# Traneptora/hydrium

Hardware: AMD Instinct MI355X
Metric: Mpixel/s encode (8K RGB, default q) (higher is better)
Workload: dtype f32

## Files before the change

hydrium_amd/csrc/hip/kernels.hip:

```cpp
#include <hip/hip_runtime.h>
#include <stdint.h>

#include "hydk_common.h"
#include <atomic>
#include <type_traits>

#pragma clang fp contract(off)

namespace {

constexpr int kThreads = 256;
#ifndef HYDK_K1_WAVES
#define HYDK_K1_WAVES 4
#endif
#ifndef HYDK_K1_GATHER
#define HYDK_K1_GATHER 0x10
#endif
#ifndef HYDK_K1_WAVELOCAL
#define HYDK_K1_WAVELOCAL 1
#endif
#ifndef HYDK_K1_SKIP
#define HYDK_K1_SKIP 0
#endif
#ifndef HYDK_K1_ILP
#define HYDK_K1_ILP 2
#endif
#ifndef HYDK_K1_TRIM
#define HYDK_K1_TRIM 0
#endif
#ifndef HYDK_K1_CHANSEQ
#define HYDK_K1_CHANSEQ 0
#endif
#ifndef HYDK_CHAIN_PROBE
#define HYDK_CHAIN_PROBE 0
#endif
#ifndef HYDK_LANE_STEP
#define HYDK_LANE_STEP 1
#endif
#ifndef HYDK_LANE_PIPE
#define HYDK_LANE_PIPE 2
#endif
#ifndef HYDK_CHAIN_PRIO
#define HYDK_CHAIN_PRIO 3
#endif
#ifndef HYDK_LANE_TAB_GLOBAL
#define HYDK_LANE_TAB_GLOBAL 0
#endif
#ifndef HYDK_CHAIN_LDS_MIN
#define HYDK_CHAIN_LDS_MIN 0
#endif
#ifndef HYDK_LANE_NC9_PROBE
#define HYDK_LANE_NC9_PROBE 9
#endif
#ifndef HYDK_CHAIN_HOG
#define HYDK_CHAIN_HOG 0
#endif
#ifndef HYDK_K1_PRIO
#define HYDK_K1_PRIO 0
#endif
constexpr int kS0Block = 72;
constexpr int kS0Chan = 32 * kS0Block;
constexpr int kDbgPitch = 2048;

constexpr float kA = (float)0.17338, kB = (float)0.146984, kC = (float)0.0982119, kD = (float)0.0344874;
constexpr float kE = (float)0.16332, kF = (float)0.0676495, kG = (float)0.125;

constexpr float kDct[7][8] = {
    {kA, kB, kC, kD, -kD, -kC, -kB, -kA},
    {kE, kF, -kF, -kE, -kE, -kF, kF, kE},
    {kB, -kD, -kA, -kC, kC, kA, kD, -kB},
    {kG, -kG, -kG, kG, kG, -kG, -kG, kG},
    {kC, -kA, kD, kB, -kB, -kD, kA, -kC},
    {kF, -kE, kE, -kF, -kF, kE, -kE, kF},
    {kD, -kC, kB, -kA, kA, -kB, kC, -kD},
};

__device__ const uint8_t kZigzag[8][8] = {
     {0, 2, 3, 9, 10, 20, 21, 35},
     {1, 4, 8, 11, 19, 22, 34, 36},
     {5, 7, 12, 18, 23, 33, 37, 48},
     {6, 13, 17, 24, 32, 38, 47, 49},
     {14, 16, 25, 31, 39, 46, 50, 57},
     {15, 26, 30, 40, 45, 51, 56, 58},
     {27, 29, 41, 44, 52, 55, 59, 62},
     {28, 42, 43, 53, 54, 60, 61, 63},
};

struct NibbleMasks {
    unsigned long long m[8][2][16];
    constexpr NibbleMasks() : m() {
        constexpr uint8_t zz[8][8] = {{0, 2, 3, 9, 10, 20, 21, 35},   {1, 4, 8, 11, 19, 22, 34, 36},  {5, 7, 12, 18, 23, 33, 37, 48},
                                      {6, 13, 17, 24, 32, 38, 47, 49}, {14, 16, 25, 31, 39, 46, 50, 57}, {15, 26, 30, 40, 45, 51, 56, 58},
                                      {27, 29, 41, 44, 52, 55, 59, 62}, {28, 42, 43, 53, 54, 60, 61, 63}};
        for (int kh = 0; kh < 8; kh++)
            for (int half = 0; half < 2; half++)
                for (int pat = 0; pat < 16; pat++) {
                    unsigned long long v = 0;
                    for (int b = 0; b < 4; b++)
                        if (pat >> b & 1)
                            v |= 1ull << zz[4 * half + b][kh];
                    m[kh][half][pat] = v;
                }
    }
};
__device__ const NibbleMasks kNibbleMasks = NibbleMasks();

__device__ const int16_t kQuantWeight[3][64] = {
    {1969, 1969, 1969, 1962, 1969, 1962, 1655, 1885, 1885, 1655, 1397, 1610, 1704, 1610, 1397, 1178,
     1368, 1494, 1494, 1368, 1178, 994,  1159, 1289, 1340, 1289, 1159, 994,  839,  980,  1104, 1178,
     1178, 1104, 980,  839,  829,  941,  1023, 1054, 1023, 941,  829,  800,  881,  928,  928,  881,
     800,  755,  809,  829,  809,  755,  663,  731,  731,  663,  491,  524,  491,  349,  349,  239},
    {280, 280, 280, 279, 280, 279, 245, 271, 271, 245, 214, 239, 250, 239, 214, 188,
     211, 226, 226, 211, 188, 164, 185, 201, 207, 201, 185, 164, 144, 163, 178, 188,
     188, 178, 163, 144, 143, 157, 168, 172, 168, 157, 143, 139, 150, 156, 156, 150,
     139, 133, 140, 143, 140, 133, 125, 129, 129, 125, 116, 118, 116, 107, 107, 98},
    {256, 147, 147, 85, 117, 85, 60, 78, 78, 60, 43, 56, 63, 56, 43, 43,
     43,  48,  48,  43, 43,  42, 43, 43, 43, 43, 43, 42, 29, 41, 43, 43,
     43,  43,  41,  29, 29,  37, 43, 43, 43, 37, 29, 27, 33, 36, 36, 33,
     27,  24,  27,  29, 27,  24, 20, 22, 22, 20, 15, 16, 15, 10, 10, 7},
};

__device__ const uint8_t kNnzCtx[64] = {
    0,   0,   31,  62,  62,  93,  93,  93,  93,  123, 123, 123, 123, 152, 152, 152, 152, 152, 152, 152, 152, 180,
    180, 180, 180, 180, 180, 180, 180, 180, 180, 180, 180, 206, 206, 206, 206, 206, 206, 206, 206, 206, 206, 206,
    206, 206, 206, 206, 206, 206, 206, 206, 206, 206, 206, 206, 206, 206, 206, 206, 206, 206, 206, 206,
};

constexpr float kLfShift[3] = {8192.f, 1024.f, 512.f};


constexpr float kUnit16 = 1.0f / (65536 - 1.0f);

__device__ __forceinline__ float linearize(float x) {
    if (x <= 0.0404482362771082f)
        return 0.07739938080495357f * x;
    return 0.003094300919832f + x * (-0.009982599f + x * (0.72007737769f + 0.2852804880f * x));
}

__device__ __forceinline__ float bias_curve(float v) {
    const float x = v + 0.0037930732552754493f;
    float z = __uint_as_float(0x548c39cbu - __float_as_uint(x) / 3u);
    z *= 1.5015480449f - 0.534850249f * x * z * z * z;
    z *= 1.333333985f - 0.33333333f * x * z * z * z;
    return 1.0f / z - 0.155954f;
}

__device__ __forceinline__ uint32_t to_u16(float x) {
    const int y = (int)(x * 65535.f + 0.5f);
    return (uint32_t)(y < 0 ? 0 : y > 65535 ? 65535 : y);
}

constexpr int kXybFastRcp = 0, kXybIeeeDiv = 1, kXybGather = 2;
constexpr int kXybFastRcpRegs = 3, kXybIeeeDivRegs = 4;
constexpr int xyb_arith(int xm) { return xm == kXybFastRcpRegs ? kXybFastRcp : xm == kXybIeeeDivRegs ? kXybIeeeDiv : xm; }
constexpr int xyb_gmask(int xm) { return xm == kXybFastRcpRegs || xm == kXybIeeeDivRegs ? 0 : HYDK_K1_GATHER; }

__device__ __forceinline__ uint32_t input_lut16_eval(uint32_t i, int linear_light) {
    const float f = (float)i * kUnit16;
    return (uint32_t)(int)((linear_light ? f : linearize(f)) * 65535.f + 0.5f);
}
constexpr uint32_t kDarkMax = 2650;
constexpr int kCurveBoth = 0, kCurveNone = 1, kCurveCubic = 2;
template <int CURVE>
__device__ __forceinline__ uint32_t input_lut16_eval_as(uint32_t i) {
    const float f = (float)i * kUnit16;
    const float y = CURVE == kCurveNone ? f : CURVE == kCurveCubic
        ? 0.003094300919832f + f * (-0.009982599f + f * (0.72007737769f + 0.2852804880f * f)) : linearize(f);
    return (uint32_t)(int)(y * 65535.f + 0.5f);
}
__device__ __forceinline__ uint32_t div3(uint32_t u) { return __umulhi(u, 0x55555556u); }
template <int XMODE>
__device__ __forceinline__ float bias_lut_eval(uint32_t i) {
    if (xyb_arith(XMODE) == kXybIeeeDiv)
        return bias_curve((float)i * kUnit16);
    const float x = (float)i * kUnit16 + 0.0037930732552754493f;
    float z = __uint_as_float(0x548c39cbu - div3(__float_as_uint(x)));
    z *= 1.5015480449f - 0.534850249f * x * z * z * z;
    z *= 1.333333985f - 0.33333333f * x * z * z * z;
    const float r0 = __builtin_amdgcn_rcpf(z);
    const float r1 = __builtin_fmaf(r0, __builtin_fmaf(-z, r0, 1.0f), r0);
    return r1 - 0.155954f;
}

#define HYDK_GLOBAL(T, p) ((__attribute__((address_space(1))) T *)(p))
template <int CURVE, int N>
__device__ __forceinline__ void input_lut16_eval_n(const uint32_t (&i)[N], uint32_t (&o)[N]) {
    float f[N], y[N];
#pragma unroll
    for (int k = 0; k < N; k++)
        f[k] = (float)i[k] * kUnit16;
    if (CURVE == kCurveNone) {
#pragma unroll
        for (int k = 0; k < N; k++)
            y[k] = f[k];
    } else {
#pragma unroll
        for (int k = 0; k < N; k++)
            y[k] = 0.2852804880f * f[k];
#pragma unroll
        for (int k = 0; k < N; k++)
            y[k] = 0.72007737769f + y[k];
#pragma unroll
        for (int k = 0; k < N; k++)
            y[k] = f[k] * y[k];
#pragma unroll
        for (int k = 0; k < N; k++)
            y[k] = -0.009982599f + y[k];
#pragma unroll
        for (int k = 0; k < N; k++)
            y[k] = f[k] * y[k];
#pragma unroll
        for (int k = 0; k < N; k++)
            y[k] = 0.003094300919832f + y[k];
        if (CURVE == kCurveBoth) {
#pragma unroll
            for (int k = 0; k < N; k++)
                y[k] = f[k] <= 0.0404482362771082f ? 0.07739938080495357f * f[k] : y[k];
        }
    }
#pragma unroll
    for (int k = 0; k < N; k++)
        y[k] = y[k] * 65535.f;
#pragma unroll
    for (int k = 0; k < N; k++)
        y[k] = y[k] + 0.5f;
#pragma unroll
    for (int k = 0; k < N; k++)
        o[k] = (uint32_t)(int)y[k];
}

template <int XMODE, int N>
__device__ __forceinline__ void bias_lut_eval_n(const uint32_t (&i)[N], float (&o)[N]) {
    if (xyb_arith(XMODE) == kXybIeeeDiv) {
#pragma unroll
        for (int k = 0; k < N; k++)
            o[k] = bias_curve((float)i[k] * kUnit16);
        return;
    }
    float x[N], z[N], t[N];
#pragma unroll
    for (int k = 0; k < N; k++)
        x[k] = (float)i[k] * kUnit16;
#pragma unroll
    for (int k = 0; k < N; k++)
        x[k] = x[k] + 0.0037930732552754493f;
#pragma unroll
    for (int k = 0; k < N; k++)
        z[k] = __uint_as_float(0x548c39cbu - div3(__float_as_uint(x[k])));
#pragma unroll
    for (int k = 0; k < N; k++)
        t[k] = 0.534850249f * x[k];
#pragma unroll
    for (int r = 0; r < 3; r++)
#pragma unroll
        for (int k = 0; k < N; k++)
            t[k] = t[k] * z[k];
#pragma unroll
    for (int k = 0; k < N; k++)
        t[k] = 1.5015480449f - t[k];
#pragma unroll
    for (int k = 0; k < N; k++)
        z[k] = z[k] * t[k];
#pragma unroll
    for (int k = 0; k < N; k++)
        t[k] = 0.33333333f * x[k];
#pragma unroll
    for (int r = 0; r < 3; r++)
#pragma unroll
        for (int k = 0; k < N; k++)
            t[k] = t[k] * z[k];
#pragma unroll
    for (int k = 0; k < N; k++)
        t[k] = 1.333333985f - t[k];
#pragma unroll
    for (int k = 0; k < N; k++)
        z[k] = z[k] * t[k];
#pragma unroll
    for (int k = 0; k < N; k++)
        t[k] = __builtin_amdgcn_rcpf(z[k]);
#pragma unroll
    for (int k = 0; k < N; k++)
        x[k] = __builtin_fmaf(-z[k], t[k], 1.0f);
#pragma unroll
    for (int k = 0; k < N; k++)
        t[k] = __builtin_fmaf(t[k], x[k], t[k]);
#pragma unroll
    for (int k = 0; k < N; k++)
        o[k] = t[k] - 0.155954f;
}

__device__ __forceinline__ uint32_t umad24(uint32_t c, uint32_t x, uint32_t acc) {
    uint32_t d;
    asm("v_mad_u32_u24 %0, %1, %2, %3" : "=v"(d) : "s"(c), "v"(x), "v"(acc));
    return d;
}

template <int XMODE>
__device__ __forceinline__ void lms_mix_u16(uint32_t r, uint32_t g, uint32_t b, const float *bias_lut, float &X,
                                            float &Y, float &B) {
    constexpr bool LUTS = XMODE == kXybGather;
    const uint32_t bb = __umul24(5112u, b);
    const uint32_t il = umad24(19661u, r, umad24(40761u, g, bb)) >> 16;
    const uint32_t im = umad24(15073u, r, umad24(45350u, g, bb)) >> 16;
    const uint32_t is = umad24(15953u, r, umad24(13419u, g, __umul24(36163u, b))) >> 16;
    float l, m, s;
    if (LUTS) {
        l = bias_lut[il];
        m = bias_lut[im];
        s = bias_lut[is];
    } else {
        const auto *gl = HYDK_GLOBAL(const float, bias_lut);
        l = (xyb_gmask(XMODE) & 8) ? gl[il] : bias_lut_eval<XMODE>(il);
        m = (xyb_gmask(XMODE) & 16) ? gl[im] : bias_lut_eval<XMODE>(im);
        s = (xyb_gmask(XMODE) & 32) ? gl[is] : bias_lut_eval<XMODE>(is);
    }
    Y = (l + m) * 0.5f;
    X = Y - m;
    B = s - Y;
}

__device__ __forceinline__ bool lms_mix_f32(float r, float g, float b, int linear_light, float &X, float &Y,
                                            float &B) {
    const bool finite = ((__float_as_uint(r) & 0x7f800000u) != 0x7f800000u) &&
                        ((__float_as_uint(g) & 0x7f800000u) != 0x7f800000u) &&
                        ((__float_as_uint(b) & 0x7f800000u) != 0x7f800000u);
    if (!linear_light) {
        r = linearize(r);
        g = linearize(g);
        b = linearize(b);
    }
    const float l = bias_curve(0.3f * r + 0.622f * g + 0.078f * b);
    const float m = bias_curve(0.23f * r + 0.692f * g + 0.078f * b);
    const float s = bias_curve(0.243423f * r + 0.204767f * g + 0.55181f * b);
    Y = (l + m) * 0.5f;
    X = Y - m;
    B = s - Y;
    return finite;
}

__device__ __forceinline__ void dct8(const float (&x)[8], float (&o)[8]) {
    float dc = x[0];
#pragma unroll
    for (int n = 1; n < 8; n++)
        dc += x[n];
    o[0] = dc * 0.125f;
#pragma unroll
    for (int k = 1; k < 8; k++) {
        if (k == 4) {
            float acc = x[0];
#pragma unroll
            for (int n = 1; n < 8; n++)
                acc = kDct[3][n] > 0 ? acc + x[n] : acc - x[n];
            o[k] = acc * 0.125f;
            continue;
        }
        float acc = x[0] * kDct[k - 1][0];
#pragma unroll
        for (int n = 1; n < 8; n++)
            acc += x[n] * kDct[k - 1][n];
        o[k] = acc;
    }
}

__device__ __forceinline__ uint32_t pack_signed(int v) {
    const uint32_t w = (uint32_t)v;
    return (w << 1) ^ (0u - (w >> 31));
}

template <int FMT>
struct SampleOf;
template <>
struct SampleOf<HYDK_FMT_U8> {
    typedef uint8_t type;
};
template <>
struct SampleOf<HYDK_FMT_U16> {
    typedef uint16_t type;
};
template <>
struct SampleOf<HYDK_FMT_F32> {
    typedef float type;
};

}

#define HYDK_URGENT() __builtin_amdgcn_s_setprio(3)

#define HYDK_DPP(v, ctrl, rmask) ((uint32_t)__builtin_amdgcn_update_dpp(0, (int)(v), (ctrl), (rmask), 0xF, false))
__device__ __forceinline__ uint32_t scan16_inclusive(uint32_t v) {
    v += HYDK_DPP(v, 0x111, 0xF);
    v += HYDK_DPP(v, 0x112, 0xF);
    v += HYDK_DPP(v, 0x114, 0xF);
    v += HYDK_DPP(v, 0x118, 0xF);
    return v;
}
__device__ __forceinline__ uint32_t scan64_inclusive(uint32_t v) {
    v = scan16_inclusive(v);
    v += HYDK_DPP(v, 0x142, 0xA);
    v += HYDK_DPP(v, 0x143, 0xC);
    return v;
}

__device__ __forceinline__ uint32_t or_reduce8(uint32_t v) {
    v |= (uint32_t)__builtin_amdgcn_update_dpp(0, (int)v, 0xB1, 0xF, 0xF, false);
    v |= (uint32_t)__builtin_amdgcn_update_dpp(0, (int)v, 0x4E, 0xF, 0xF, false);
    v |= (uint32_t)__builtin_amdgcn_update_dpp(0, (int)v, 0x141, 0xF, 0xF, false);
    return v;
}

template <int FMT>
__device__ __forceinline__ void store_record(void *tok, uint32_t at, uint32_t token, uint32_t cluster, uint32_t symbol,
                                             uint32_t rbits, uint32_t residue) {
    if (FMT == HYDK_FMT_F32)
        ((uint64_t *)tok)[at] = ((uint64_t)residue << 32) | HYDK_REC_LO(token, cluster, rbits);
    else {
#if HYDK_K1_TRIM
        const uint32_t off = at * 4u;
        *(HYDK_GLOBAL(uint32_t, (char *)tok + off)) = HYDK_REC32(symbol, rbits, residue);
#else
        HYDK_GLOBAL(uint32_t, tok)[at] = HYDK_REC32(symbol, rbits, residue);
#endif
    }
}

template <int FMT>
__device__ __forceinline__ int trunc_as_reference(float x) {
    const int q = (int)x;
    if (FMT != HYDK_FMT_F32)
        return q;
    return x < 2147483648.0f ? q : (int)0x80000000u;
}

#define HYDK_K1_OCCUPANCY __launch_bounds__(kThreads, HYDK_K1_WAVES)
template <int FMT, int XMODE, int STORE = HYDK_STORE_F32>
__global__ HYDK_K1_OCCUPANCY void k_transform_tokenize(const HydkLfJob *__restrict__ jobs, uint32_t *status, uint2 *part_info,
                                                       int plog) {
    static_assert(STORE == HYDK_STORE_F32 || (STORE == HYDK_STORE_NV12 ? FMT == HYDK_FMT_U8 : FMT == HYDK_FMT_F32),
                  "the float class has the half-precision storage forms, the 8-bit class NV12");
    constexpr bool NV12 = STORE == HYDK_STORE_NV12;
    constexpr bool HALF = STORE != HYDK_STORE_F32 && !NV12;
    typedef typename std::conditional<HALF, uint16_t, typename SampleOf<FMT>::type>::type sample_t;
    constexpr bool LUTS = XMODE == kXybGather;
    constexpr int kWords = FMT == HYDK_FMT_U8 ? 6 : 12;
#if HYDK_K1_PRIO
    __builtin_amdgcn_s_setprio(HYDK_K1_PRIO);
#endif
    const unsigned bid = blockIdx.x >> plog, part = blockIdx.x & ((1u << plog) - 1u);
    const HydkLfJob job = jobs[bid >> 6];
    if (job.fmt != FMT || (FMT != HYDK_FMT_F32 && job.use_luts != xyb_arith(XMODE) + (NV12 ? HYDK_VARIANT_NV12 : 0)) ||
        (FMT == HYDK_FMT_F32 && job.storage != (uint32_t)STORE))
        return;
    if ((int)(bid & 63) >= job.gcols * job.grows)
        return;
    if (FMT == HYDK_FMT_F32 && job.rec_bytes != 8) {
        if (threadIdx.x == 0) {
            atomicOr(status, HYDK_STATUS_LAYOUT);
            job.sym_count[bid & 63] = 0;
            job.rbits_total[bid & 63] = 0;
            if (plog)
                part_info[blockIdx.x] = uint2{0u, 0u};
        }
        return;
    }

#if HYDK_K1_CHANSEQ
    static_assert(HYDK_K1_WAVELOCAL, "the channels share one row-pass buffer: a wavefront must read only what it wrote");
    typedef typename std::conditional<FMT == HYDK_FMT_F32, int32_t, int16_t>::type coef_t;
    constexpr int kQBlock = 64;
    __shared__ float s_rowpass[kS0Chan];
    __shared__ __attribute__((aligned(16))) coef_t s_q[3 * 32 * kQBlock];
#else
    __shared__ float s_rowpass[3 * kS0Chan];
#endif
    __shared__ uint32_t s_boff[33];
    __shared__ uint32_t s_rbits;
    constexpr int kHistW = FMT == HYDK_FMT_F32 ? 72 : (int)HYDK_REC32_TOKENS;
    __shared__ uint32_t s_hist[HYDK_MAX_CLUSTERS * kHistW];
    __shared__ uint16_t s_lut8[256];
    __shared__ uint8_t s_nnz3[64];
    __shared__ uint16_t s_jinfo[64];
    __shared__ uint4 s_seg[32 * 3];
    __shared__ uint32_t s_blen[32];
    __shared__ __attribute__((aligned(16))) float s_wq[3 * 64];

    const int t = threadIdx.x;
    const int lane = t & 63;
    const int wave = t >> 6;
    const int g = (int)(bid & 63);
    const int gx = g % job.gcols, gy = g / job.gcols;
    const int px0 = gx << 8, py0 = gy << 8;
    const int gw = min(256, job.width - px0), gh = min(256, job.height - py0);
    const int gbw = (gw + 7) >> 3, gbh = (gh + 7) >> 3;

    for (int i = t; i < HYDK_MAX_CLUSTERS * kHistW; i += kThreads)
        s_hist[i] = 0;
    if (FMT == HYDK_FMT_U8)
        s_lut8[t] = job.in_lut8[t];
    if (t < 64) {
        const int j = t;
        s_nnz3[t] = kNnzCtx[t] % 3;
        ((uint8_t *)s_jinfo)[2 * kZigzag[t >> 3][t & 7]] = HYDK_K1_CHANSEQ ? (uint8_t)(((t & 7) << 3) | (t >> 3)) : (uint8_t)t;
        ((uint8_t *)s_jinfo)[2 * t + 1] = (uint8_t)((j < 2 ? 0 : j < 16 ? j - 1 : j < 32 ? 15 + ((j - 16) >> 1) : 23 + ((j - 32) >> 2)) % 3);
    }
    if (t < 192)
        s_wq[t] = (float)kQuantWeight[t >> 6][kZigzag[t & 7][(t >> 3) & 7]];

    const int cb = t >> 3, kh = t & 7;
    const uint32_t nib_row = (uint32_t)kh * (uint32_t)sizeof(kNibbleMasks.m[0]);
    const int coef_cl_lo = job.scheme == 0 ? 3 : job.scheme == 3 ? 0 : 1;

    const bool packed = !NV12 && job.pixel_stride == 3 &&
                        (const char *)job.src[1] == (const char *)job.src[0] + sizeof(sample_t) &&
                        (const char *)job.src[2] == (const char *)job.src[0] + 2 * sizeof(sample_t) &&
                        (((uintptr_t)job.src[0] | (uintptr_t)(job.row_stride * (long long)sizeof(sample_t))) & 3) == 0 &&
                        FMT != HYDK_FMT_F32;

#if HYDK_K1_WAVELOCAL
    const int ar = lane >> 3, ab = (wave << 3) | (lane & 7);
#else
    const int ar = t >> 5, ab = t & 31;
#endif
    int hrun = 0;
    if (HALF) {
        const bool rows4 = ((job.row_stride * 2) & 3) == 0;
        if (!(job.per_sample & 1u) && job.pixel_stride == 3 && rows4 && ((uintptr_t)job.src[0] & 3) == 0 &&
            (const char *)job.src[1] == (const char *)job.src[0] + 2 && (const char *)job.src[2] == (const char *)job.src[0] + 4)
            hrun = 1;
        else if (!(job.per_sample & 2u) && job.pixel_stride == 1 && rows4 &&
                 (((uintptr_t)job.src[0] | (uintptr_t)job.src[1] | (uintptr_t)job.src[2]) & 3) == 0)
            hrun = 2;
    }
    const bool hfast = HALF && hrun != 0 && ab < gbw && ab * 8 + 8 <= gw;
    const bool nvrun = NV12 && (((uintptr_t)job.src[0] | (uintptr_t)job.src[1] | (uintptr_t)job.row_stride) & 3) == 0;
    const HydkYuvMatrix yuv = hydk_yuv_matrix(NV12 ? (int)job.matrix : 0);
    const bool fast = (NV12 ? nvrun : packed) && ab < gbw && ab * 8 + 8 <= gw;
    uint32_t nxt[kWords];
#pragma unroll
    for (int k = 0; k < kWords; k++)
        nxt[k] = 0;
    auto prefetch = [&](int s) {
        if (HALF) {
            if (hfast && s * 8 + ar < gh) {
                const long long row = (long long)(py0 + s * 8 + ar) * job.row_stride;
                if (hrun == 1) {
                    const char *p = (const char *)job.src[0] + (row + (long long)(px0 + ab * 8) * 3) * 2;
#pragma unroll
                    for (int k = 0; k < 12; k++)
                        nxt[k] = HYDK_GLOBAL(const uint32_t, p)[k];
                } else {
#pragma unroll
                    for (int c = 0; c < 3; c++) {
                        const char *p = (const char *)job.src[c] + (row + (long long)(px0 + ab * 8)) * 2;
#pragma unroll
                        for (int k = 0; k < 4; k++)
                            nxt[4 * c + k] = HYDK_GLOBAL(const uint32_t, p)[k];
                    }
                }
            }
            return;
        }
        if (NV12) {
            if (fast && s * 8 + ar < gh) {
                const long long y = py0 + s * 8 + ar, x = px0 + ab * 8;
                const char *py = (const char *)job.src[0] + y * job.row_stride + x;
                const char *pc = (const char *)job.src[1] + (y >> 1) * job.row_stride + x;
#pragma unroll
                for (int k = 0; k < 2; k++) {
                    nxt[k] = HYDK_GLOBAL(const uint32_t, py)[k];
                    nxt[2 + k] = HYDK_GLOBAL(const uint32_t, pc)[k];
                }
            }
            return;
        }
        if (fast && s * 8 + ar < gh) {
            const uint32_t *p = (const uint32_t *)((const char *)job.src[0] +
                                                   ((long long)(py0 + s * 8 + ar) * job.row_stride +
                                                    (long long)(px0 + ab * 8) * 3) * (long long)sizeof(sample_t));
#pragma unroll
            for (int k = 0; k < kWords; k++)
                nxt[k] = HYDK_GLOBAL(const uint32_t, p)[k];
        }
    };
    const int s_per = (gbh + (1 << plog) - 1) >> plog;
    const int s_first = (int)part * s_per, s_end = min(gbh, s_first + s_per);
    const uint32_t tok_room = job.tok_cap >> plog;
    prefetch(s_first);

    void *const tok = (char *)job.tokens + (size_t)g * job.tok_cap * job.rec_bytes + (size_t)part * tok_room * (FMT == HYDK_FMT_F32 ? 8u : 4u);
    uint32_t goff = 0;
    uint32_t rb_sum = 0;
    bool overflowed = false;
    if (t == 0)
        s_rbits = 0;
    bool bad_sample = false;
    __syncthreads();

    for (int s = s_first; s < s_end; s++) {
        float xv[8], yv[8], bv[8];
        if (ab < gbw) {
            const int y = py0 + s * 8 + ar;
            const int x0 = px0 + ab * 8;
            const bool row_ok = s * 8 + ar < gh;
            auto float_pixel = [&](float fr, float fg, float fb, float &X, float &Y, float &B) {
                if (job.bad_slot) {
                    const bool ir = (__float_as_uint(fr) & 0x7f800000u) == 0x7f800000u;
                    const bool ig = (__float_as_uint(fg) & 0x7f800000u) == 0x7f800000u;
                    const bool ib = (__float_as_uint(fb) & 0x7f800000u) == 0x7f800000u;
                    bad_sample = bad_sample || ir || ig || ib;
                    fr = ir ? 0.0f : fr;
                    fg = ig ? 0.0f : fg;
                    fb = ib ? 0.0f : fb;
                }
                if (!lms_mix_f32(fr, fg, fb, job.linear_light, X, Y, B))
                    bad_sample = true;
            };
            if (HALF && hfast) {
#pragma unroll
                for (int i = 0; i < 8; i++) {
                    xv[i] = yv[i] = bv[i] = 0.0f;
                    if (row_ok) {
                        float f[3];
#pragma unroll
                        for (int ch = 0; ch < 3; ch++) {
                            const int ki = i * 3 + ch, kp = ch * 8 + i;
                            const uint32_t wi = nxt[ki >> 1] >> (16 * (ki & 1)), wp = nxt[kp >> 1] >> (16 * (kp & 1));
                            f[ch] = __uint_as_float(hydk_widen_half(STORE, (hrun == 1 ? wi : wp) & 0xFFFFu));
                        }
                        float_pixel(f[0], f[1], f[2], xv[i], yv[i], bv[i]);
                    }
                }
                prefetch(s + 1);
            } else if (fast) {
                uint32_t cvt[kWords];
                if (NV12) {
#pragma unroll
                    for (int k = 0; k < kWords; k++)
                        cvt[k] = 0;
#pragma unroll
                    for (int i = 0; i < 8; i++) {
                        uint32_t rgb[3];
                        hydk_yuv_to_rgb(yuv, (nxt[i >> 2] >> (8 * (i & 3))) & 0xFF, (nxt[2 + (i >> 2)] >> (8 * (i & 2))) & 0xFF,
                                        (nxt[2 + (i >> 2)] >> (8 * (i & 2) + 8)) & 0xFF, rgb);
#pragma unroll
                        for (int ch = 0; ch < 3; ch++) {
                            const int si = i * 3 + ch;
                            cvt[si >> 2] |= rgb[ch] << (8 * (si & 3));
                        }
                    }
                }
                uint32_t(&w)[kWords] = NV12 ? cvt : nxt;
                int curve = kCurveBoth;
                if (FMT == HYDK_FMT_U16 && !LUTS) {
                    if (job.linear_light)
                        curve = kCurveNone;
                    else {
                        typedef uint16_t u16x2 __attribute__((ext_vector_type(2)));
                        u16x2 mn = __builtin_bit_cast(u16x2, w[0]);
#pragma unroll
                        for (int k = 1; k < kWords; k++)
                            mn = __builtin_elementwise_min(mn, __builtin_bit_cast(u16x2, w[k]));
                        const bool dark = row_ok && (uint32_t)(mn.x < mn.y ? mn.x : mn.y) <= kDarkMax;
                        curve = __builtin_amdgcn_ballot_w64(dark) ? kCurveBoth : kCurveCubic;
                    }
                }
                auto row_to_xyb = [&](auto curve_tag) {
                    constexpr int CURVE = decltype(curve_tag)::value;
#if HYDK_K1_ILP
                    if (FMT != HYDK_FMT_F32 && !LUTS) {
                        constexpr int P = HYDK_K1_ILP;
#pragma unroll
                        for (int i0 = 0; i0 < 8; i0 += P) {
                            uint32_t smp[3 * P], lin[3 * P], idx[3 * P];
                            float bia[3 * P];
                            if (FMT == HYDK_FMT_U8) {
#pragma unroll
                                for (int k = 0; k < 3 * P; k++) {
                                    const int si = i0 * 3 + k;
                                    lin[k] = s_lut8[(w[si >> 2] >> (8 * (si & 3))) & 0xFF];
                                }
                            } else {
#pragma unroll
                                for (int k = 0; k < 3 * P; k++) {
                                    const int si = i0 * 3 + k;
                                    smp[k] = (w[si >> 1] >> (16 * (si & 1))) & 0xFFFF;
                                }
                                input_lut16_eval_n<CURVE, 3 * P>(smp, lin);
                            }
#pragma unroll
                            for (int q = 0; q < P; q++) {
                                const uint32_t r = lin[3 * q], g = lin[3 * q + 1], b = lin[3 * q + 2];
                                const uint32_t bb = __umul24(5112u, b);
                                idx[3 * q] = umad24(19661u, r, umad24(40761u, g, bb)) >> 16;
                                idx[3 * q + 1] = umad24(15073u, r, umad24(45350u, g, bb)) >> 16;
                                idx[3 * q + 2] = umad24(15953u, r, umad24(13419u, g, __umul24(36163u, b))) >> 16;
                            }
                            constexpr auto gathered = [](int k) constexpr { return ((xyb_gmask(XMODE) >> 3) >> (k % 3) & 1) != 0; };
                            constexpr int NG = [&]() constexpr { int n = 0; for (int k = 0; k < 3 * P; k++) n += gathered(k); return n; }();
                            if (NG == 0)
                                bias_lut_eval_n<XMODE, 3 * P>(idx, bia);
                            else {
                                const auto *gl = HYDK_GLOBAL(const float, job.bias_lut);
                                constexpr int NE = 3 * P - NG > 0 ? 3 * P - NG : 1;
                                uint32_t eidx[NE];
                                float eb[NE];
                                int n = 0;
#pragma unroll
                                for (int k = 0; k < 3 * P; k++) {
                                    if (gathered(k))
                                        bia[k] = gl[idx[k]];
                                    else
                                        eidx[n++] = idx[k];
                                }
                                if (NG < 3 * P)
                                    bias_lut_eval_n<XMODE, NE>(eidx, eb);
                                n = 0;
#pragma unroll
                                for (int k = 0; k < 3 * P; k++)
                                    if (!gathered(k))
                                        bia[k] = eb[n++];
                            }
#pragma unroll
                            for (int q = 0; q < P; q++) {
                                const float Y = (bia[3 * q] + bia[3 * q + 1]) * 0.5f;
                                yv[i0 + q] = Y;
                                xv[i0 + q] = Y - bia[3 * q + 1];
                                bv[i0 + q] = bia[3 * q + 2] - Y;
                            }
                        }
                        return;
                    }
#endif
#pragma unroll
                    for (int i = 0; i < 8; i++) {
                        uint32_t rgb[3];
#pragma unroll
                        for (int ch = 0; ch < 3; ch++) {
                            const int si = i * 3 + ch;
                            if (FMT == HYDK_FMT_U8)
                                rgb[ch] = s_lut8[(w[si >> 2] >> (8 * (si & 3))) & 0xFF];
                            else {
                                const uint32_t v = (w[si >> 1] >> (16 * (si & 1))) & 0xFFFF;
                                rgb[ch] = LUTS ? (uint32_t)job.in_lut16[v] : (xyb_gmask(XMODE) >> ch & 1) ? (uint32_t)HYDK_GLOBAL(const uint16_t, job.in_lut16)[v] : input_lut16_eval_as<CURVE>(v);
                            }
                        }
                        if (HYDK_K1_SKIP & 2) {
                            xv[i] = __uint_as_float(0x3f000000u | w[(i * 3) >> 1]);
                            yv[i] = __uint_as_float(0x3f000000u | w[(i * 3 + 1) >> 1]);
                            bv[i] = __uint_as_float(0x3f000000u | w[(i * 3 + 2) >> 1]);
                            continue;
                        }
                        lms_mix_u16<XMODE>(rgb[0], rgb[1], rgb[2], job.bias_lut, xv[i], yv[i], bv[i]);
                    }
                };
                if (row_ok) {
                    if (curve == kCurveCubic)
                        row_to_xyb(std::integral_constant<int, kCurveCubic>());
                    else if (curve == kCurveNone)
                        row_to_xyb(std::integral_constant<int, kCurveNone>());
                    else
                        row_to_xyb(std::integral_constant<int, kCurveBoth>());
                } else {
#pragma unroll
                    for (int i = 0; i < 8; i++)
                        xv[i] = yv[i] = bv[i] = 0.0f;
                }
                prefetch(s + 1);
            } else {
                const int nvalid = row_ok ? min(8, gw - ab * 8) : 0;
#pragma unroll
                for (int i = 0; i < 8; i++) {
                    xv[i] = yv[i] = bv[i] = 0.0f;
                    if (i < nvalid) {
                        const long long off = (long long)y * job.row_stride + (long long)(x0 + i) * job.pixel_stride;
                        const long long offc = NV12 ? (long long)(y >> 1) * job.row_stride + (long long)((x0 + i) & ~1) : off;
                        const sample_t sr = ((const sample_t *)job.src[0])[off];
                        const sample_t sg = ((const sample_t *)job.src[1])[offc];
                        const sample_t sb = ((const sample_t *)job.src[2])[offc];
                        if (FMT == HYDK_FMT_F32) {
                            float fr, fg, fb;
                            if (HALF) {
                                fr = __uint_as_float(hydk_widen_half(STORE, (uint32_t)sr));
                                fg = __uint_as_float(hydk_widen_half(STORE, (uint32_t)sg));
                                fb = __uint_as_float(hydk_widen_half(STORE, (uint32_t)sb));
                            } else {
                                fr = (float)sr, fg = (float)sg, fb = (float)sb;
                            }
                            float_pixel(fr, fg, fb, xv[i], yv[i], bv[i]);
                        } else {
                            uint32_t rgb[3] = {(uint32_t)sr, (uint32_t)sg, (uint32_t)sb};
                            if (NV12)
                                hydk_yuv_to_rgb(yuv, (uint32_t)sr, (uint32_t)sg, (uint32_t)sb, rgb);
#pragma unroll
                            for (int ch = 0; ch < 3; ch++) {
                                if (FMT == HYDK_FMT_U8)
                                    rgb[ch] = s_lut8[rgb[ch]];
                                else
                                    rgb[ch] = LUTS ? job.in_lut16[rgb[ch]] : input_lut16_eval(rgb[ch], job.linear_light);
                            }
                            lms_mix_u16<XMODE>(rgb[0], rgb[1], rgb[2], job.bias_lut, xv[i], yv[i], bv[i]);
                        }
                    }
                }
            }
            if (job.dbg_xyb) {
                float *d = job.dbg_xyb + (size_t)y * kDbgPitch + x0;
#pragma unroll
                for (int i = 0; i < 8; i++) {
                    d[i] = xv[i];
                    d[(size_t)kDbgPitch * kDbgPitch + i] = yv[i];
                    d[(size_t)2 * kDbgPitch * kDbgPitch + i] = bv[i];
                }
            }
#if !HYDK_K1_CHANSEQ
            float o[8];
            float *dst = s_rowpass + ab * kS0Block + ar * 8;
            dct8(xv, o);
#pragma unroll
            for (int k = 0; k < 8; k++)
                dst[k] = o[k];
            dct8(yv, o);
#pragma unroll
            for (int k = 0; k < 8; k++)
                dst[kS0Chan + k] = o[k];
            dct8(bv, o);
#pragma unroll
            for (int k = 0; k < 8; k++)
                dst[2 * kS0Chan + k] = o[k];
#endif
        }
#define HYDK_K1_WAVE_SYNC()                                                                                      \
    do {                                                                                                         \
        __builtin_amdgcn_fence(__ATOMIC_RELEASE, "wavefront");                                                   \
        __builtin_amdgcn_wave_barrier();                                                                         \
        __builtin_amdgcn_fence(__ATOMIC_ACQUIRE, "wavefront");                                                   \
    } while (0)
#if HYDK_K1_CHANSEQ
#elif HYDK_K1_WAVELOCAL
        HYDK_K1_WAVE_SYNC();
#else
        __syncthreads();
#endif

        unsigned long long msk[3] = {0, 0, 0};
        int32_t lf_int[3] = {0, 0, 0};
        auto column_pass = [&](const int c) __attribute__((always_inline)) {
                float col[8], v[8];
                float *src = s_rowpass + (HYDK_K1_CHANSEQ ? 0 : c * kS0Chan) + cb * kS0Block + kh;
#pragma unroll
                for (int n = 0; n < 8; n++)
                    col[n] = src[n * 8];
                dct8(col, v);
                if (job.dbg_dct) {
                    float *d = job.dbg_dct + (size_t)c * kDbgPitch * kDbgPitch +
                               (size_t)(py0 + s * 8 + kh) * kDbgPitch + px0 + cb * 8;
#pragma unroll
                    for (int kv = 0; kv < 8; kv++)
                        d[kv] = v[kv];
                }
                uint32_t nlo = 0, nhi = 0;
                int q[8];
                const float4 w03 = *(const float4 *)&s_wq[c * 64 + kh * 8], w47 = *(const float4 *)&s_wq[c * 64 + kh * 8 + 4];
                const float wq[8] = {w03.x, w03.y, w03.z, w03.w, w47.x, w47.y, w47.z, w47.w};
#pragma unroll
                for (int kv = 0; kv < 8; kv++) {
                    const float scaled = v[kv] * wq[kv] * 5.0f;
                    int qq = trunc_as_reference<FMT>(scaled);
                    const bool nz = (FMT == HYDK_FMT_F32 ? !(__builtin_fabsf(scaled) < 2.0f) : __builtin_fabsf(scaled) >= 2.0f) &&
                                    !(kv == 0 && kh == 0);
                    qq = nz ? qq : 0;
                    q[kv] = qq;
                    if (kv < 4)
                        nlo |= nz ? 8u << kv : 0u;
                    else
                        nhi |= nz ? 8u << (kv - 4) : 0u;
#if !HYDK_K1_CHANSEQ
                    ((int *)src)[kv * 8] = qq;
#endif
                }
#if HYDK_K1_CHANSEQ
                {
                    coef_t *const dq = s_q + (c * 32 + cb) * kQBlock + kh * 8;
                    if (FMT == HYDK_FMT_F32) {
                        *(int4 *)dq = int4{q[0], q[1], q[2], q[3]};
                        *(int4 *)(dq + 4) = int4{q[4], q[5], q[6], q[7]};
                    } else {
                        const uint32_t k0 = 0x05040100u;
                        *(uint4 *)dq = uint4{__builtin_amdgcn_perm((uint32_t)q[1], (uint32_t)q[0], k0), __builtin_amdgcn_perm((uint32_t)q[3], (uint32_t)q[2], k0),
                                             __builtin_amdgcn_perm((uint32_t)q[5], (uint32_t)q[4], k0), __builtin_amdgcn_perm((uint32_t)q[7], (uint32_t)q[6], k0)};
                    }
                }
#endif
                if (job.dbg_quant) {
                    int32_t *d = job.dbg_quant + (size_t)c * kDbgPitch * kDbgPitch +
                                 (size_t)(py0 + s * 8 + kh) * kDbgPitch + px0 + cb * 8;
#pragma unroll
                    for (int kv = 0; kv < 8; kv++)
                        d[kv] = q[kv];
                }
                const char *const nib = (const char *)&kNibbleMasks.m[0][0][0];
                if (!(HYDK_K1_SKIP & 4))
                msk[c] = *(const unsigned long long *)(nib + (nib_row | nlo)) | *(const unsigned long long *)(nib + (nib_row | 128u | nhi));
                lf_int[c] = trunc_as_reference<FMT>(v[0] * kLfShift[c]);
        };
#if HYDK_K1_CHANSEQ
        {
#pragma unroll
            for (int c = 0; c < 3; c++) {
                if (ab < gbw) {
                    float o[8];
                    float *dst = s_rowpass + ab * kS0Block + ar * 8;
                    if (c == 0)
                        dct8(xv, o);
                    else if (c == 1)
                        dct8(yv, o);
                    else
                        dct8(bv, o);
#pragma unroll
                    for (int k = 0; k < 8; k++)
                        dst[k] = o[k];
                }
                HYDK_K1_WAVE_SYNC();
                if (!(HYDK_K1_SKIP & 8) && cb < gbw)
                    column_pass(c);
                HYDK_K1_WAVE_SYNC();
            }
        }
#endif
        if (!(HYDK_K1_SKIP & 8) && cb < gbw) {
#if !HYDK_K1_CHANSEQ
#pragma unroll
            for (int c = 0; c < 3; c++)
                column_pass(c);
#endif
            if (kh == 0) {
#pragma unroll
                for (int c = 0; c < 3; c++)
                    HYDK_GLOBAL(int32_t, job.dc)[(size_t)c * HYDK_DC_PITCH * HYDK_DC_PITCH + (size_t)((py0 >> 3) + s) * HYDK_DC_PITCH + (px0 >> 3) + cb] = lf_int[c];
            }
#if HYDK_K1_TRIM & 2
            {
                typedef unsigned long long u64;
                u64 *const cell = (u64 *)&s_seg[cb * 3];
                if (kh == 0) {
                    cell[0] = 0;
                    cell[2] = 0;
                    cell[4] = 0;
                }
                __builtin_amdgcn_wave_barrier();
                constexpr int at[3] = {2, 0, 4};
#pragma unroll
                for (int c = 0; c < 3; c++) {
                    __hip_atomic_fetch_or((uint32_t *)&cell[at[c]], (uint32_t)msk[c], __ATOMIC_RELAXED, __HIP_MEMORY_SCOPE_WORKGROUP);
                    __hip_atomic_fetch_or((uint32_t *)&cell[at[c]] + 1, (uint32_t)(msk[c] >> 32), __ATOMIC_RELAXED, __HIP_MEMORY_SCOPE_WORKGROUP);
                }
                __builtin_amdgcn_wave_barrier();
                if (kh == 0) {
#pragma unroll
                    for (int c = 0; c < 3; c++)
                        msk[c] = cell[at[c]];
                }
            }
#else
#pragma unroll
            for (int c = 0; c < 3 && !(HYDK_K1_SKIP & 4); c++) {
                const uint32_t lo = or_reduce8((uint32_t)msk[c]), hi = or_reduce8((uint32_t)(msk[c] >> 32));
                msk[c] = ((unsigned long long)hi << 32) | lo;
            }
#endif
        }
        const uint32_t nY = 1u + (msk[1] ? 63u - (uint32_t)__clzll(msk[1]) : 0u);
        const uint32_t nX = 1u + (msk[0] ? 63u - (uint32_t)__clzll(msk[0]) : 0u);
        const uint32_t nB = 1u + (msk[2] ? 63u - (uint32_t)__clzll(msk[2]) : 0u);
        if (kh == 0) {
            s_blen[cb] = cb < gbw ? nY | (nX << 8) | (nB << 16) : 0u;
#if HYDK_K1_CHANSEQ
            const uint32_t base = (uint32_t)(cb * kQBlock), chan_pitch = 32u * kQBlock;
#else
            const uint32_t base = (uint32_t)(cb * kS0Block), chan_pitch = (uint32_t)kS0Chan;
#endif
            s_seg[cb * 3 + 0] = make_uint4((uint32_t)msk[1], (uint32_t)(msk[1] >> 32), nY | ((uint32_t)__popcll(msk[1]) << 8), base + chan_pitch);
            s_seg[cb * 3 + 1] = make_uint4((uint32_t)msk[0], (uint32_t)(msk[0] >> 32), nX | ((uint32_t)__popcll(msk[0]) << 8), base);
            s_seg[cb * 3 + 2] = make_uint4((uint32_t)msk[2], (uint32_t)(msk[2] >> 32), nB | ((uint32_t)__popcll(msk[2]) << 8), base + 2 * chan_pitch);
        }
        __syncthreads();

        {
            const uint32_t len3 = s_blen[lane & 31];
            const uint32_t mine = (len3 & 0xffu) + ((len3 >> 8) & 0xffu) + (len3 >> 16);
            uint32_t inc = scan16_inclusive(mine);
            inc += HYDK_DPP(inc, 0x142, 0xA);
            s_boff[(lane & 31) + 1] = inc;
            if (lane == 0)
                s_boff[0] = 0;
            __builtin_amdgcn_wave_barrier();
        }
        const uint32_t strip_total = s_boff[32];

        {
            overflowed = overflowed || goff + strip_total > tok_room;
            static_assert(kThreads == 256, "run lengths are computed with shifts");
            const uint32_t per = strip_total >> 8, extra = strip_total & 255u;
            uint32_t p = (uint32_t)t * per + min((uint32_t)t, extra);
            const uint32_t pend = overflowed ? 0u : p + per + ((uint32_t)t < extra ? 1u : 0u);
            if (!(HYDK_K1_SKIP & 1) && p < pend) {
                uint32_t b = 0;
#pragma unroll
                for (uint32_t step = 16; step; step >>= 1)
                    b += s_boff[b + step] <= p ? step : 0u;
                uint32_t j = p - s_boff[b];
                const uint32_t len = s_blen[b];
                uint32_t visit = 0;
                if (j >= (len & 0xffu)) {
                    j -= len & 0xffu;
                    visit = 1;
                    if (j >= ((len >> 8) & 0xffu)) {
                        j -= (len >> 8) & 0xffu;
                        visit = 2;
                    }
                }
                uint32_t seg_at = b * 3u + visit;
                uint4 seg = s_seg[seg_at];
                uint32_t n = seg.z & 0xffu, nz_total = seg.z >> 8;
                const unsigned long long m = ((unsigned long long)seg.y << 32) | seg.x;
                uint32_t remaining = nz_total - (uint32_t)__popcll(m & ((1ull << j) - 1ull));
                uint32_t prev = j <= 1u ? (uint32_t)(nz_total <= 4u) : (uint32_t)(m >> (j - 1u)) & 1u;
                const uint32_t coef_base = (uint32_t)coef_cl_lo;
                const uint32_t prev_mask = job.scheme <= 1 ? 1u : 0u, ctx_mask = job.scheme == 0 ? 6u : 0u;
                const uint32_t count_mask = job.scheme == 0 ? 3u : 0u;
                for (; p < pend; p++) {
                    const uint32_t ji = s_jinfo[j];
#if HYDK_K1_CHANSEQ
                    const int coef = (int)s_q[seg.w + (ji & 0xffu)];
#else
                    const int coef = ((const int *)s_rowpass)[seg.w + (ji & 0xffu)];
#endif
                    const bool is_count = j == 0u;
                    const uint32_t value = is_count ? nz_total : pack_signed(coef);
                    const uint32_t u = visit + (uint32_t)s_nnz3[remaining & 63u] + (ji >> 8);
                    const uint32_t cluster = is_count ? (visit & count_mask)
                                                      : coef_base + (prev & prev_mask) + ((0x1248u >> (u + u)) & ctx_mask);
                    uint32_t token, rbits, residue;
                    if (FMT != HYDK_FMT_F32) {
                        const uint32_t fb = __float_as_uint((float)value) >> 22;
                        const bool big = value >= 16u;
                        token = big ? fb - 246u : value;
                        rbits = big ? (fb >> 1) - 128u : 0u;
                        residue = __builtin_amdgcn_ubfe(value, 0u, rbits);
                    } else if (value < 16) {
                        token = value;
                        rbits = 0;
                        residue = 0;
                    } else {
                        const int nb = 30 - __clz((int)value);
                        rbits = (uint32_t)nb;
                        residue = value & ((1u << nb) - 1u);
                        token = 16u + (((uint32_t)(nb - 3) << 1) | ((value >> nb) & 1u));
                    }
#if HYDK_K1_TRIM
                    const uint32_t bin = umad24(cluster, (uint32_t)kHistW, FMT == HYDK_FMT_F32 ? min(token, (uint32_t)kHistW - 1u) : token);
#else
                    const uint32_t bin = cluster * kHistW + (FMT == HYDK_FMT_F32 ? min(token, (uint32_t)kHistW - 1u) : token);
#endif
                    store_record<FMT>(tok, goff + p, token, cluster, bin, rbits, residue);
                    rb_sum += rbits;
                    atomicAdd(&s_hist[bin], 1u);
                    const uint32_t here = coef != 0 ? 1u : 0u;
                    remaining -= here;
                    prev = is_count ? (uint32_t)(nz_total <= 4u) : here;
                    if (++j == n) {
                        seg_at++;
                        visit = visit == 2u ? 0u : visit + 1u;
                        seg = s_seg[seg_at];
                        n = seg.z & 0xffu;
                        nz_total = remaining = seg.z >> 8;
                        j = 0;
                    }
                }
            }
        }
        goff += strip_total;
        __syncthreads();
    }

    __syncthreads();
    uint32_t top_token = 0;
    for (int i = t; i < HYDK_MAX_CLUSTERS * kHistW; i += kThreads) {
        const uint32_t v = s_hist[i];
        if (v) {
            atomicAdd(&job.hist[(i / kHistW) * HYDK_ALPHABET + i % kHistW], v);
            top_token = max(top_token, (uint32_t)(i % kHistW) + 1u);
        }
    }
#pragma unroll
    for (int d = 32; d; d >>= 1)
        top_token = max(top_token, (uint32_t)__shfl_xor((int)top_token, d));
    if (lane == 0 && top_token)
        atomicMax(job.alpha_max, top_token);
#pragma unroll
    for (int d = 32; d; d >>= 1)
        rb_sum += (uint32_t)__shfl_xor((int)rb_sum, d);
    if (lane == 0)
        atomicAdd(&s_rbits, rb_sum);
    __syncthreads();
    if (t == 0) {
        const uint32_t count = overflowed || HYDK_K1_SKIP ? 0u : goff;
        if (plog) {
            part_info[blockIdx.x] = uint2{count, s_rbits};
        } else {
            job.sym_count[g] = count;
            job.rbits_total[g] = s_rbits;
        }
        if (overflowed)
            atomicOr(status, HYDK_STATUS_TOKENS);
    }
    if (FMT == HYDK_FMT_F32 && bad_sample) {
        if (job.bad_slot)
            atomicOr(job.bad_slot, 1u);
        else
            atomicOr(status, HYDK_STATUS_BAD_SAMPLE);
    }
}

#include "lf_huffman.h"

__global__ __launch_bounds__(kThreads) void k_join_parts(const HydkLfJob *__restrict__ jobs, const uint2 *part_info, int plog,
                                                         uint32_t *status) {
    const HydkLfJob job = jobs[blockIdx.x >> 6];
    const int g = blockIdx.x & 63;
    if (g >= job.gcols * job.grows)
        return;
    const uint32_t parts = 1u << plog, room = job.tok_cap >> plog, wpr = job.fmt == HYDK_FMT_F32 ? 2u : 1u;
    uint32_t *const base = (uint32_t *)((char *)job.tokens + (size_t)g * job.tok_cap * job.rec_bytes);
    bool bogus = false;
    uint2 p0 = part_info[(size_t)blockIdx.x * parts];
    if (p0.x > room) {
        p0 = uint2{0u, 0u};
        bogus = true;
    }
    uint32_t total = p0.x, rbits = p0.y;
    for (uint32_t q = 1; q < parts; q++) {
        uint2 pi = part_info[(size_t)blockIdx.x * parts + q];
        if (pi.x > room) {
            pi = uint2{0u, 0u};
            bogus = true;
        }
        const uint32_t *src = base + (size_t)q * room * wpr;
        uint32_t *dst = base + (size_t)total * wpr;
        const uint32_t words = pi.x * wpr;
        if (dst != src) {
            constexpr uint32_t kPer = 8;
            for (uint32_t at = 0; at < words; at += kPer * kThreads) {
                uint32_t v[kPer];
#pragma unroll
                for (uint32_t k = 0; k < kPer; k++) {
                    const uint32_t i = at + k * kThreads + threadIdx.x;
                    v[k] = i < words ? src[i] : 0u;
                }
                __syncthreads();
#pragma unroll
                for (uint32_t k = 0; k < kPer; k++) {
                    const uint32_t i = at + k * kThreads + threadIdx.x;
                    if (i < words)
                        dst[i] = v[k];
                }
            }
        }
        total += pi.x;
        rbits += pi.y;
    }
    if (threadIdx.x == 0) {
        job.sym_count[g] = bogus ? 0u : total;
        job.rbits_total[g] = bogus ? 0u : rbits;
        if (bogus)
            atomicOr(status, HYDK_STATUS_INCONSISTENT);
    }
}

__global__ __launch_bounds__(kThreads) void k_build_tables(const uint32_t *hist_all, HydkTables *tabs,
                                                           const uint32_t *alpha_max_all, int nclusters,
                                                           uint32_t alpha_floor, const uint32_t *alpha_floor_dev,
                                                           int first_slot, int num_slots, const uint32_t *lf_hist,
                                                           HydkLfStream *lf_streams, void *lf_work, const HydkLfJob *__restrict__ jobs_all) {
    HYDK_URGENT();
    if ((int)blockIdx.x >= num_slots) {
        __shared__ LfHuffScratch s_huff;
        const int s = (int)blockIdx.x - num_slots;
        if (threadIdx.x < 64)
            lf_huffman_wave(lf_hist + (size_t)s * HYDK_LF_CODES, ((LfWork *)lf_work)[s].codes, lf_streams + s, s_huff, (int)threadIdx.x);
        return;
    }
    const unsigned slot = (unsigned)first_slot + blockIdx.x;
    const uint32_t *hist = hist_all + (size_t)slot * HYDK_MAX_CLUSTERS * HYDK_ALPHABET;
    HydkTables *tab = tabs + slot;
    __shared__ uint32_t s_freq[HYDK_MAX_CLUSTERS][HYDK_ALPHABET];
    __shared__ uint32_t s_cutoff[HYDK_MAX_CLUSTERS][HYDK_ALPHABET];
    __shared__ uint32_t s_other[HYDK_MAX_CLUSTERS][HYDK_ALPHABET];
    __shared__ uint32_t s_shift[HYDK_MAX_CLUSTERS][HYDK_ALPHABET];
    __shared__ uint32_t s_base[HYDK_MAX_CLUSTERS][HYDK_ALPHABET];
    __shared__ uint8_t s_under[HYDK_MAX_CLUSTERS][HYDK_ALPHABET];
    __shared__ uint8_t s_over[HYDK_MAX_CLUSTERS][HYDK_ALPHABET];
    __shared__ uint32_t s_alpha[HYDK_MAX_CLUSTERS];
    __shared__ uint32_t s_log_alpha, s_err;

    const int t = threadIdx.x;
    for (int i = t; i < HYDK_MAX_CLUSTERS * HYDK_ALPHABET; i += kThreads) {
// ... 1517 lines not shown
```

Baseline: 99580.

## Use butterfly column DCT with exact fallback near quantization boundaries

For integer input formats, the column DCT now uses a butterfly even/odd decomposition with FMAs, folds the 5x scale into the quant weights, and computes an error band from the column's absolute sum. If any coefficient falls close to an integer rounding boundary within that band, the exact reference-order dot product is recomputed for it, with wave-uniform ballot branches. The goal is to cut per-column ALU work while keeping bit-exact quantized output. The cost is extra band and boundary checks plus occasional divergent recompute, and it relies on the error bound being correct.

```diff
diff --git a/hydrium_amd/csrc/hip/hydk_column.h b/hydrium_amd/csrc/hip/hydk_column.h
--- /dev/null
+++ b/hydrium_amd/csrc/hip/hydk_column.h
@@ -0,0 +1,99 @@
+#pragma once
+
+#include <math.h>
+
+#ifdef __HIPCC__
+#define HYD_COL_FN __host__ __device__ static inline __attribute__((always_inline))
+#else
+#define HYD_COL_FN static inline __attribute__((always_inline))
+#endif
+
+constexpr float kA = (float)0.17338, kB = (float)0.146984, kC = (float)0.0982119, kD = (float)0.0344874;
+constexpr float kE = (float)0.16332, kF = (float)0.0676495, kG = (float)0.125;
+
+constexpr float kDct[7][8] = {
+    {kA, kB, kC, kD, -kD, -kC, -kB, -kA},
+    {kE, kF, -kF, -kE, -kE, -kF, kF, kE},
+    {kB, -kD, -kA, -kC, kC, kA, kD, -kB},
+    {kG, -kG, -kG, kG, kG, -kG, -kG, kG},
+    {kC, -kA, kD, kB, -kB, -kD, kA, -kC},
+    {kF, -kE, kE, -kF, -kF, kE, -kE, kF},
+    {kD, -kC, kB, -kA, kA, -kB, kC, -kD},
+};
+
+HYD_COL_FN void dct8(const float (&x)[8], float (&o)[8]) {
+    float dc = x[0];
+#pragma unroll
+    for (int n = 1; n < 8; n++)
+        dc += x[n];
+    o[0] = dc * 0.125f;
+#pragma unroll
+    for (int k = 1; k < 8; k++) {
+        if (k == 4) {
+            float acc = x[0];
+#pragma unroll
+            for (int n = 1; n < 8; n++)
+                acc = kDct[3][n] > 0 ? acc + x[n] : acc - x[n];
+            o[k] = acc * 0.125f;
+            continue;
+        }
+        float acc = x[0] * kDct[k - 1][0];
+#pragma unroll
+        for (int n = 1; n < 8; n++)
+            acc += x[n] * kDct[k - 1][n];
+        o[k] = acc;
+    }
+}
+
+HYD_COL_FN float hyd_col_exact(const float (&x)[8], const int k) {
+    if (k == 0 || k == 4) {
+        float acc = x[0];
+#pragma unroll
+        for (int n = 1; n < 8; n++)
+            acc = (k == 0 || kDct[3][n] > 0) ? acc + x[n] : acc - x[n];
+        return acc * 0.125f;
+    }
+    float acc = x[0] * kDct[k - 1][0];
+#pragma unroll
+    for (int n = 1; n < 8; n++)
+        acc += x[n] * kDct[k - 1][n];
+    return acc;
+}
+
+HYD_COL_FN void hyd_col_fast(const float (&x)[8], float (&o)[8]) {
+    const float d0 = x[0] - x[7], d1 = x[1] - x[6], d2 = x[2] - x[5], d3 = x[3] - x[4];
+    const float s0 = x[0] + x[7], s1 = x[1] + x[6], s2 = x[2] + x[5], s3 = x[3] + x[4];
+    const float p = s0 - s3, q = s1 - s2;
+    o[1] = fmaf(d3, kD, fmaf(d2, kC, fmaf(d1, kB, d0 * kA)));
+    o[3] = fmaf(d3, -kC, fmaf(d2, -kA, fmaf(d1, -kD, d0 * kB)));
+    o[5] = fmaf(d3, kB, fmaf(d2, kD, fmaf(d1, -kA, d0 * kC)));
+    o[7] = fmaf(d3, -kA, fmaf(d2, kB, fmaf(d1, -kC, d0 * kD)));
+    o[2] = fmaf(q, kF, p * kE);
+    o[6] = fmaf(q, -kE, p * kF);
+}
+
+constexpr float kColBand = kA * 48.0f * 5.9604644775390625e-08f;
+
+HYD_COL_FN float hyd_col_band(const float (&x)[8]) {
+    float sum = fabsf(x[0]);
+#pragma unroll
+    for (int n = 1; n < 8; n++)
+        sum += fabsf(x[n]);
+    return sum * kColBand;
+}
+
+HYD_COL_FN float hyd_col_fract(const float t) {
+#if defined(__HIP_DEVICE_COMPILE__)
+    return __builtin_amdgcn_fractf(t);
+#else
+    return t - floorf(t);
+#endif
+}
+
+HYD_COL_FN bool hyd_col_undecided(const float s_fast, const float w5, const float band) {
+    const float eps2 = band * w5;
+    const float t = fmaf(eps2, 0.5f, fabsf(s_fast));
+    return t >= 2.0f && hyd_col_fract(t) < eps2;
+}
+
+HYD_COL_FN float hyd_col_weight(const float w5) { return w5 * 0.2f; }
diff --git a/hydrium_amd/csrc/hip/kernels.hip b/hydrium_amd/csrc/hip/kernels.hip
--- a/hydrium_amd/csrc/hip/kernels.hip
+++ b/hydrium_amd/csrc/hip/kernels.hip
@@ -7,6 +7,8 @@
 
 #pragma clang fp contract(off)
 
+#include "hydk_column.h"
+
 namespace {
 
 constexpr int kThreads = 256;
@@ -61,19 +63,6 @@
 constexpr int kS0Block = 72;
 constexpr int kS0Chan = 32 * kS0Block;
 constexpr int kDbgPitch = 2048;
-
-constexpr float kA = (float)0.17338, kB = (float)0.146984, kC = (float)0.0982119, kD = (float)0.0344874;
-constexpr float kE = (float)0.16332, kF = (float)0.0676495, kG = (float)0.125;
-
-constexpr float kDct[7][8] = {
-    {kA, kB, kC, kD, -kD, -kC, -kB, -kA},
-    {kE, kF, -kF, -kE, -kE, -kF, kF, kE},
-    {kB, -kD, -kA, -kC, kC, kA, kD, -kB},
-    {kG, -kG, -kG, kG, kG, -kG, -kG, kG},
-    {kC, -kA, kD, kB, -kB, -kD, kA, -kC},
-    {kF, -kE, kE, -kF, -kF, kE, -kE, kF},
-    {kD, -kC, kB, -kA, kA, -kB, kC, -kD},
-};
 
 __device__ const uint8_t kZigzag[8][8] = {
      {0, 2, 3, 9, 10, 20, 21, 35},
@@ -338,30 +327,6 @@
     return finite;
 }
 
-__device__ __forceinline__ void dct8(const float (&x)[8], float (&o)[8]) {
-    float dc = x[0];
-#pragma unroll
-    for (int n = 1; n < 8; n++)
-        dc += x[n];
-    o[0] = dc * 0.125f;
-#pragma unroll
-    for (int k = 1; k < 8; k++) {
-        if (k == 4) {
-            float acc = x[0];
-#pragma unroll
-            for (int n = 1; n < 8; n++)
-                acc = kDct[3][n] > 0 ? acc + x[n] : acc - x[n];
-            o[k] = acc * 0.125f;
-            continue;
-        }
-        float acc = x[0] * kDct[k - 1][0];
-#pragma unroll
-        for (int n = 1; n < 8; n++)
-            acc += x[n] * kDct[k - 1][n];
-        o[k] = acc;
-    }
-}
-
 __device__ __forceinline__ uint32_t pack_signed(int v) {
     const uint32_t w = (uint32_t)v;
     return (w << 1) ^ (0u - (w >> 31));
@@ -502,8 +467,10 @@
         ((uint8_t *)s_jinfo)[2 * kZigzag[t >> 3][t & 7]] = HYDK_K1_CHANSEQ ? (uint8_t)(((t & 7) << 3) | (t >> 3)) : (uint8_t)t;
         ((uint8_t *)s_jinfo)[2 * t + 1] = (uint8_t)((j < 2 ? 0 : j < 16 ? j - 1 : j < 32 ? 15 + ((j - 16) >> 1) : 23 + ((j - 32) >> 2)) % 3);
     }
-    if (t < 192)
-        s_wq[t] = (float)kQuantWeight[t >> 6][kZigzag[t & 7][(t >> 3) & 7]];
+    if (t < 192) {
+        const float w = (float)kQuantWeight[t >> 6][kZigzag[t & 7][(t >> 3) & 7]];
+        s_wq[t] = FMT != HYDK_FMT_F32 && (t & 3) ? w * 5.0f : w;
+    }
 
     const int cb = t >> 3, kh = t & 7;
     const uint32_t nib_row = (uint32_t)kh * (uint32_t)sizeof(kNibbleMasks.m[0]);
@@ -849,21 +816,69 @@
 #pragma unroll
                 for (int n = 0; n < 8; n++)
                     col[n] = src[n * 8];
-                dct8(col, v);
+                if (FMT == HYDK_FMT_F32) {
+                    dct8(col, v);
+                } else {
+                    v[0] = hyd_col_exact(col, 0);
+                    hyd_col_fast(col, v);
+                }
+                const float dc = v[0];
+                const float band = FMT == HYDK_FMT_F32 ? 0.0f : hyd_col_band(col);
                 if (job.dbg_dct) {
                     float *d = job.dbg_dct + (size_t)c * kDbgPitch * kDbgPitch +
                                (size_t)(py0 + s * 8 + kh) * kDbgPitch + px0 + cb * 8;
+                    float dv[8];
+                    if (FMT == HYDK_FMT_F32) {
+#pragma unroll
+                        for (int kv = 0; kv < 8; kv++)
+                            dv[kv] = v[kv];
+                    } else {
+                        float cx[8];
+#pragma unroll
+                        for (int n = 0; n < 8; n++) {
+                            cx[n] = col[n];
+                            asm volatile("" : "+v"(cx[n]));
+                        }
+                        dct8(cx, dv);
+                    }
 #pragma unroll
                     for (int kv = 0; kv < 8; kv++)
-                        d[kv] = v[kv];
+                        d[kv] = dv[kv];
                 }
                 uint32_t nlo = 0, nhi = 0;
                 int q[8];
                 const float4 w03 = *(const float4 *)&s_wq[c * 64 + kh * 8], w47 = *(const float4 *)&s_wq[c * 64 + kh * 8 + 4];
                 const float wq[8] = {w03.x, w03.y, w03.z, w03.w, w47.x, w47.y, w47.z, w47.w};
+                float sc[8];
+                if (FMT == HYDK_FMT_F32) {
+#pragma unroll
+                    for (int kv = 0; kv < 8; kv++)
+                        sc[kv] = v[kv] * wq[kv] * 5.0f;
+                } else {
+                    sc[0] = v[0] * wq[0] * 5.0f;
+                    sc[4] = hyd_col_exact(col, 4) * wq[4] * 5.0f;
+                    bool undecided[8], any = false;
+#pragma unroll
+                    for (int kv = 1; kv < 8; kv++) {
+                        if (kv == 4)
+                            continue;
+                        sc[kv] = v[kv] * wq[kv];
+                        undecided[kv] = hyd_col_undecided(sc[kv], wq[kv], band);
+                        any |= undecided[kv];
+                    }
+                    if (__builtin_amdgcn_ballot_w64(any) != 0) {
+#pragma unroll
+                        for (int kv = 1; kv < 8; kv++) {
+                            if (kv == 4)
+                                continue;
+                            if (__builtin_amdgcn_ballot_w64(undecided[kv]) != 0)
+                                sc[kv] = hyd_col_exact(col, kv) * hyd_col_weight(wq[kv]) * 5.0f;
+                        }
+                    }
+                }
 #pragma unroll
                 for (int kv = 0; kv < 8; kv++) {
-                    const float scaled = v[kv] * wq[kv] * 5.0f;
+                    const float scaled = sc[kv];
                     int qq = trunc_as_reference<FMT>(scaled);
                     const bool nz = (FMT == HYDK_FMT_F32 ? !(__builtin_fabsf(scaled) < 2.0f) : __builtin_fabsf(scaled) >= 2.0f) &&
                                     !(kv == 0 && kh == 0);
@@ -900,7 +915,7 @@
                 const char *const nib = (const char *)&kNibbleMasks.m[0][0][0];
                 if (!(HYDK_K1_SKIP & 4))
                 msk[c] = *(const unsigned long long *)(nib + (nib_row | nlo)) | *(const unsigned long long *)(nib + (nib_row | 128u | nhi));
-                lf_int[c] = trunc_as_reference<FMT>(v[0] * kLfShift[c]);
+                lf_int[c] = trunc_as_reference<FMT>(dc * kLfShift[c]);
         };
 #if HYDK_K1_CHANSEQ
         {
```

Measured after the change: 100,200 (median of 6 runs). No clear change (+0.6%).
